# 10258392511/InverseProblemWithDiffusionModel

Hardware: AMD Instinct MI355X
Metric: ALD reconstructions/sec (128x128 complex, R=40, 4-coil) (higher is better)
Workload: dtype f32 (convolutions: operands as two fp16 pieces = 22 significand bits + 2 signs, three fp16 MFMAs per product, fp32 accumulate; every image scaled into fp16's range by an exact power of two from its producer's per-image maxima: any fp32 input, DESIGN.md 4.2); 1 GPU; ACDC-style 128x128 complex SENSE R=40 4-coil ALD reconstruction, NCSNv2Deepest ngf=128 (94.1M params, seeded random init), sigma 348->0.01 x 2311 levels x 3 steps, L2Penalty, denoise; 14 posterior samples = 14 on rank 0 + 13 per further rank (the 105-sample / 8-GPU partition of BASELINE config 3); samples_total=14, samples_this_rank=14, parallelism=sample-sharded x1, hip_graph=True, state_finite=True

## Files before the change

include/ipdm.h:

```cpp
#ifndef IPDM_H
#define IPDM_H

#include <stddef.h>
#include <stdint.h>

#ifdef __cplusplus
extern "C" {
#endif

#define IPDM_OK 0
#define IPDM_EINVAL (-1)
#define IPDM_EUNSUPPORTED (-2)

#define IPDM_ACT_NONE 0
#define IPDM_ACT_ELU 1
#define IPDM_ACT_RELU 2
#define IPDM_ACT_LRELU02 3
#define IPDM_ACT_SWISH 4
#define IPDM_ACT_COPY 5

#define IPDM_AMAX_WAYS 8
#define IPDM_AMAX_SLOT 128

#define IPDM_ABI_VERSION 4
// ... 235 lines not shown
int ipdm_ndft_forward_sets_c64(const float* x, const float* sens, const double* traj, int traj_sets, float* y, float* work,
                               int B, int n_coils, int M, int H, int W, void* stream);
int ipdm_ndft_adjoint_sets_c64(const float* y, const float* sens, const double* traj, int traj_sets, const float* weights,
                               float* x, float* work, int B, int n_coils, int M, int H, int W, void* stream);
int ipdm_toeplitz_psf_sets_f32(const double* traj, int traj_sets, const float* weights, float* psf, float* work, int M, int H,
                               int W, void* stream);
int ipdm_toeplitz_normal_sets_c64(const float* v, const float* sens, const float* psf, int psf_sets, float* out, float* work,
                                  int B, int n_coils, int H, int W, void* stream);
int ipdm_nc_sense_cgprox_sets_f32(const float* z_re, const float* z_im, const float* sens, const float* psf, int psf_sets,
                                  float a, const float* ahy, int max_iter, float tol, float* out_re, float* out_im,
                                  float* work, int32_t* iters_out, int B, int n_coils, int H, int W, void* stream);
int ipdm_ald_nc_sense_cg_step_sets_f32(float* x_re, float* x_im, const float* g_re, const float* g_im,
                                       const float* noise_re, const float* noise_im,
                                       float step, float noise_scale, uint64_t seed, int64_t sample_offset, int64_t step_id,
                                       const ipdm_sched_t* dev_sched, int sched_stride, const float* sens, const float* psf,
                                       int psf_sets, float coef, float* work, const float* ahy, int max_iter, float tol,
                                       int32_t* iters_out, int B, int n_coils, int H, int W, void* stream);

size_t ipdm_nc_coil_gram_workspace_bytes(int B, int n_coils, int M);
int ipdm_nc_coil_gram_c64(const float* y, const float* weights, float* gram, float* work, int B, int n_coils, int M, void* stream);

int ipdm_langevin_step_f32(float* x, const float* g, const float* noise, float step, float noise_scale,
                           uint64_t seed, int64_t sample_offset, int64_t step_id, const ipdm_sched_t* dev_sched,
                           int64_t n_samples, int64_t sample_elems, void* stream);

int ipdm_philox_normal_f32(float* out, uint64_t seed, int64_t sample_offset, int64_t step_id, int plane,
                           int64_t n_samples, int64_t sample_elems, void* stream);

int ipdm_philox_block_host(uint64_t seed, int64_t sample, int64_t step_id, int plane, uint32_t quad, uint32_t* out4);


int ipdm_instnorm_plus_coef_f32(const float* x, const float* alpha, const float* gamma, const float* beta,
                                float* coef, int B, int C, int HW,
                                float* amax_bound ,
                                void* stream);
int ipdm_cond_instnorm_plus_coef_f32(const float* x, const float* embed, const int64_t* labels, int num_classes, int bias,
                                     float* coef, int B, int C, int HW, float* amax_bound, void* stream);
int ipdm_affine_act_f32(const float* x, const float* coef, float* y, int B, int C, int HW, int act, void* stream);
int ipdm_act_f32(const float* x, float* y, int64_t n, int act, void* stream);
int ipdm_scale_shift_f32(const float* x, float* y, int64_t n, float a, float b, void* stream);
int ipdm_add_f32(const float* x, const float* y, float* out, int64_t n, void* stream);
int ipdm_div_sigma_f32(const float* x, const float* sigmas, const int64_t* labels, float* out,
                       int B, int64_t sample_elems, void* stream);
int ipdm_conv3x3_thin_supported(int Cin, int Cout, int H, int W);
int ipdm_conv3x3_thin_f32(const float* x, const float* w, const float* bias,
                          const float* coef ,
                          float* out, int B, int Cin, int Cout, int H, int W, void* stream);
int ipdm_conv3x3_thin_stats_partials(int Cin, int Cout, int H, int W);
int ipdm_conv3x3_thin_stats_f32(const float* x, const float* w, const float* bias, const float* coef, float* out, float* part,
                                int B, int Cin, int Cout, int H, int W, void* stream);
int ipdm_conv3x3_fewout_fin_supported(int Cin, int Cout, int H, int W);
int ipdm_conv3x3_fewout_fin_f32(const float* x, const float* w, const float* bias, const float* coef, int act, float* out,
                                int B, int Cin, int Cout, int H, int W, void* stream);
int ipdm_maxpool5_f32(const float* x, float* y, int planes, int H, int W, void* stream);
int ipdm_affine_avgpool5_f32(const float* x, const float* coef, float* y, int planes, int H, int W, void* stream);
int ipdm_meanpool2_f32(const float* x, float* y, int planes, int H, int W, void* stream);
int ipdm_bilinear_f32(const float* x, float* out, int planes, int in_h, int in_w, int out_h, int out_w,
                      int accumulate, int act ,
                      int planes_per_image, float* amax_out ,
                      void* stream);
int ipdm_trilinear_f32(const float* x, float* out, int planes, int in_d, int in_h, int in_w, int out_d, int out_h,
                       int out_w, int accumulate, int act, int planes_per_image, float* amax_out, void* stream);

int ipdm_groupnorm_coef_f32(const float* x, const float* weight, const float* bias, float* coef,
                            int B, int C, int HW, int G, float eps,
                            float* plane_amax ,
                            void* stream);
int ipdm_groupnorm_coef_partials_f32(const float* part1, int C1, const float* part2, int C2, int P, const float* weight,
                                     const float* bias, float* coef , int B, int G, float eps, void* stream);
int ipdm_groupnorm_coef_cat_f32(const float* x1, int C1, const float* x2, int C2, const float* weight, const float* bias,
                                float* coef, int B, int HW, int G, float eps, float* plane_amax ,
                                void* stream);
int ipdm_affine_act_cat_f32(const float* x1, int C1, const float* x2, int C2, const float* coef, float* y, int B, int HW,
                            int act, void* stream);
int ipdm_linear_f32(const float* x, const float* W, const float* bias, float* y, int B, int In, int Out,
                    int act, void* stream);
int ipdm_attention_f32(const float* q, const float* k, const float* v, float* out, int B, int C, int N,
                       float scale, void* stream);
int ipdm_axpby_f32(const float* x, const float* y, float* out, int64_t n, float a, float b, void* stream);
int ipdm_sample_axpy2_f32(const float* x, const float* y, const float* z, const float* a, const float* c,
                          float* out, int n_samples, int64_t sample_elems, void* stream);
int ipdm_sample_norm_f32(const float* x, float* norms, int n_samples, int64_t sample_elems, void* stream);

int ipdm_conv_pack_weight_f32(const float* w , float* wt, int Cout, int Cin, int k, void* stream);
int ipdm_conv2d_f32(const float* x, const float* wt, const float* bias, const float* coef, int act,
                    const float* residual, float* out, float* out_act, int act_out,
                    int B, int Cin, int Cout, int H, int W, int k, int dilation, int pool2, void* stream);

int ipdm_conv_wino_weight_f32(const float* w , float* U, int Cout, int Cin, void* stream);
int ipdm_conv2d_wino_supported(int Cin, int Cout, int H, int W, int dilation);
int ipdm_conv2d_wino_f32(const float* x, const float* U, const float* bias, const float* residual, float* out,
                         float* out_act, int act_out, int B, int Cin, int Cout, int H, int W, int dilation,
                         void* stream);

int ipdm_debug_set_stamp_buffer(void* buf);
int64_t ipdm_debug_lds_optin_count(void);

int ipdm_conv3d_f32(const float* x, const float* wt, const float* bias, const float* coef, int act,
                    const float* residual, float* out, float* out_act, int act_out,
                    int B, int Cin, int Cout, int D, int H, int W, int k, int dilation, void* stream);

int ipdm_maxpool3d5_f32(const float* x, float* y, int planes, int D, int H, int W, void* stream);
int ipdm_temporal_taps_f32(const float* x, float* out, int planes, int S, int T_in, int T_out, int mode, void* stream);

typedef struct {
  const float* in_amax;
// ... 135 lines not shown
```

inverseproblemwithdiffusionmodel_amd/_lib.py:

```python
import ctypes
import os

import torch
from ctypes import c_char_p, c_double, c_float, c_int, c_int64, c_uint64, c_void_p


class ConvExt(ctypes.Structure):
    _fields_ = [("in_amax", c_void_p), ("bias_bstride", c_int), ("out_scale", c_float), ("res_second", c_int),
                ("out_amax", c_void_p), ("act_amax", c_void_p)]


_HERE = os.path.dirname(os.path.abspath(__file__))
LIB_PATH = os.environ.get("IPDM_LIB") or os.path.join(_HERE, "libipdm.so")

P = c_void_p

SIGNATURES = {
    "ipdm_abi_version": [],
    "ipdm_build_arch": [],
    "ipdm_upfirdn2d_f32": [P, P, P] + [c_int] * 14 + [P],
    "ipdm_fused_bias_act_f32": [P, P, P, P, c_int64, c_int, c_int, c_int, c_int, c_float, c_float, P],
    "ipdm_upfirdn2d_f16": [P, P, P] + [c_int] * 14 + [P],
    "ipdm_upfirdn2d_f64": [P, P, P] + [c_int] * 14 + [P],
    "ipdm_fused_bias_act_f16": [P, P, P, P, c_int64, c_int, c_int, c_int, c_int, c_float, c_float, P],
# ... 59 lines not shown
    "ipdm_ald_singlecoil_step_f32": [P, P, P, P, P, P, c_float, c_float, c_uint64, c_int64, c_int64, P,
                                     P, P, c_int, c_float, c_int, P, c_int, c_int, c_int, P],
    "ipdm_pc_langevin_coef_workspace_bytes": [c_int],
    "ipdm_pc_langevin_coef_f32": [P, P, P, P, c_double, c_double, c_uint64, c_int64, c_int64, P, c_float, c_float, P, P,
                                  c_int, c_int64, P],
    "ipdm_pc_sense_step_f32": [P, P, P, P, P, P, c_float, c_float, c_uint64, c_int64, c_int64, P, c_int,
                               P, P, c_int, c_int, P, c_int, c_float, P, c_int, c_int, c_int, c_int, P],
    "ipdm_pc_sense_cg_step_f32": [P, P, P, P, P, P, c_float, c_float, c_uint64, c_int64, c_int64, P, c_int,
                                  P, P, c_int, c_int, P, c_int, c_float, P, P, c_int, c_float, P,
                                  c_int, c_int, c_int, c_int, P],
    "ipdm_pc_singlecoil_step_f32": [P, P, P, P, P, P, c_float, c_float, c_uint64, c_int64, c_int64, P, c_int,
                                    P, P, c_int, c_float, c_int, P, c_int, c_int, c_int, P],
    "ipdm_nc_supported": [c_int, c_int],
    "ipdm_ndft_workspace_bytes": [c_int, c_int, c_int],
    "ipdm_ndft_forward_c64": [P, P, P, P, P, c_int, c_int, c_int, c_int, c_int, P],
    "ipdm_ndft_adjoint_c64": [P, P, P, P, P, P, c_int, c_int, c_int, c_int, c_int, P],
    "ipdm_toeplitz_psf_workspace_bytes": [c_int, c_int, c_int],
    "ipdm_toeplitz_psf_f32": [P, P, P, P, c_int, c_int, c_int, P],
    "ipdm_toeplitz_workspace_bytes": [c_int, c_int, c_int, c_int],
    "ipdm_toeplitz_normal_c64": [P, P, P, P, P, c_int, c_int, c_int, c_int, P],
    "ipdm_nc_sense_cg_workspace_bytes": [c_int, c_int, c_int, c_int],
    "ipdm_nc_sense_cgprox_f32": [P, P, P, P, c_float, P, c_int, c_float, P, P, P, P, c_int, c_int, c_int, c_int, P],
    "ipdm_ald_nc_sense_cg_step_f32": [P, P, P, P, P, P, c_float, c_float, c_uint64, c_int64, c_int64, P, c_int,
                                      P, P, c_float, P, P, c_int, c_float, P, c_int, c_int, c_int, c_int, P],
    "ipdm_ndft_forward_sets_c64": [P, P, P, c_int, P, P, c_int, c_int, c_int, c_int, c_int, P],
    "ipdm_ndft_adjoint_sets_c64": [P, P, P, c_int, P, P, P, c_int, c_int, c_int, c_int, c_int, P],
    "ipdm_toeplitz_psf_sets_f32": [P, c_int, P, P, P, c_int, c_int, c_int, P],
    "ipdm_toeplitz_normal_sets_c64": [P, P, P, c_int, P, P, c_int, c_int, c_int, c_int, P],
    "ipdm_nc_sense_cgprox_sets_f32": [P, P, P, P, c_int, c_float, P, c_int, c_float, P, P, P, P, c_int, c_int, c_int, c_int, P],
    "ipdm_ald_nc_sense_cg_step_sets_f32": [P, P, P, P, P, P, c_float, c_float, c_uint64, c_int64, c_int64, P, c_int,
                                           P, P, c_int, c_float, P, P, c_int, c_float, P, c_int, c_int, c_int, c_int, P],
    "ipdm_nc_coil_gram_workspace_bytes": [c_int, c_int, c_int],
    "ipdm_nc_coil_gram_c64": [P, P, P, P, c_int, c_int, c_int, P],
    "ipdm_langevin_step_f32": [P, P, P, c_float, c_float, c_uint64, c_int64, c_int64, P, c_int64, c_int64, P],
    "ipdm_philox_normal_f32": [P, c_uint64, c_int64, c_int64, c_int, c_int64, c_int64, P],
    "ipdm_philox_block_host": [c_uint64, c_int64, c_int64, c_int, ctypes.c_uint32, P],
    "ipdm_instnorm_plus_coef_f32": [P, P, P, P, P, c_int, c_int, c_int, P, P],
    "ipdm_cond_instnorm_plus_coef_f32": [P, P, P, c_int, c_int, P, c_int, c_int, c_int, P, P],
    "ipdm_affine_act_f32": [P, P, P, c_int, c_int, c_int, c_int, P],
    "ipdm_act_f32": [P, P, c_int64, c_int, P],
    "ipdm_scale_shift_f32": [P, P, c_int64, c_float, c_float, P],
    "ipdm_add_f32": [P, P, P, c_int64, P],
    "ipdm_div_sigma_f32": [P, P, P, P, c_int, c_int64, P],
    "ipdm_maxpool5_f32": [P, P, c_int, c_int, c_int, P],
    "ipdm_affine_avgpool5_f32": [P, P, P, c_int, c_int, c_int, P],
    "ipdm_meanpool2_f32": [P, P, c_int, c_int, c_int, P],
    "ipdm_bilinear_f32": [P, P, c_int, c_int, c_int, c_int, c_int, c_int, c_int, c_int, P, P],
    "ipdm_conv3x3_thin_supported": [c_int, c_int, c_int, c_int],
    "ipdm_conv3x3_thin_f32": [P, P, P, P, P, c_int, c_int, c_int, c_int, c_int, P],
    "ipdm_conv3x3_thin_stats_partials": [c_int, c_int, c_int, c_int],
    "ipdm_conv3x3_thin_stats_f32": [P, P, P, P, P, P, c_int, c_int, c_int, c_int, c_int, P],
    "ipdm_conv3x3_fewout_fin_supported": [c_int, c_int, c_int, c_int],
    "ipdm_conv3x3_fewout_fin_f32": [P, P, P, P, c_int, P, c_int, c_int, c_int, c_int, c_int, P],
    "ipdm_trilinear_f32": [P, P, c_int, c_int, c_int, c_int, c_int, c_int, c_int, c_int, c_int, c_int, P, P],
    "ipdm_groupnorm_coef_f32": [P, P, P, P, c_int, c_int, c_int, c_int, c_float, P, P],
    "ipdm_groupnorm_coef_partials_f32": [P, c_int, P, c_int, c_int, P, P, P, c_int, c_int, c_float, P],
    "ipdm_groupnorm_coef_cat_f32": [P, c_int, P, c_int, P, P, P, c_int, c_int, c_int, c_float, P, P],
    "ipdm_affine_act_cat_f32": [P, c_int, P, c_int, P, P, c_int, c_int, c_int, P],
    "ipdm_linear_f32": [P, P, P, P, c_int, c_int, c_int, c_int, P],
    "ipdm_attention_f32": [P, P, P, P, c_int, c_int, c_int, c_float, P],
    "ipdm_axpby_f32": [P, P, P, c_int64, c_float, c_float, P],
    "ipdm_sample_axpy2_f32": [P, P, P, P, P, P, c_int, c_int64, P],
    "ipdm_sample_norm_f32": [P, P, c_int, c_int64, P],
    "ipdm_conv_pack_weight_f32": [P, P, c_int, c_int, c_int, P],
    "ipdm_conv2d_f32": [P, P, P, P, c_int, P, P, P, c_int] + [c_int] * 8 + [P],
    "ipdm_conv_wino_weight_f32": [P, P, c_int, c_int, P],
    "ipdm_conv2d_wino_supported": [c_int, c_int, c_int, c_int, c_int],
    "ipdm_conv2d_wino_f32": [P, P, P, P, P, P, c_int, c_int, c_int, c_int, c_int, c_int, c_int, P],
    "ipdm_debug_set_stamp_buffer": [P],
    "ipdm_debug_lds_optin_count": [],
    "ipdm_conv3d_f32": [P, P, P, P, c_int, P, P, P, c_int] + [c_int] * 8 + [P],
    "ipdm_maxpool3d5_f32": [P, P, c_int, c_int, c_int, c_int, P],
    "ipdm_temporal_taps_f32": [P, P, c_int, c_int, c_int, c_int, c_int, P],
    "ipdm_conv_bx3_weight_bytes": [c_int, c_int, c_int],
    "ipdm_conv_bx3_pack_weight": [P, P, c_int, c_int, c_int, P],
    "ipdm_conv2d_bx3_f32": [P, P, P, P, c_int, P, P, P, c_int] + [c_int] * 7 + [P, P],
    "ipdm_conv3d_bx3_f32": [P, P, P, P, c_int, P, P, P, c_int] + [c_int] * 8 + [P, P],
    "ipdm_conv_bx3_splitk": [c_int] * 8,
    "ipdm_conv_bx3_splitk_f32": [P, P, P, P, c_int, P, P, P, c_int] + [c_int] * 10 + [P, P, P],
    "ipdm_adam_ascent_f32": [P, P, P, P, c_int64, c_float, c_float, c_float, c_float, c_int, P],
    "ipdm_conv_wino_bx3_weight_bytes": [c_int, c_int],
    "ipdm_conv_wino_bx3_pack_weight": [P, P, c_int, c_int, P],
    "ipdm_conv2d_wino_bx3_supported": [c_int, c_int, c_int, c_int, c_int],
    "ipdm_conv2d_wino_bx3_f32": [P, P, P, P, P, P, c_int, c_int, c_int, c_int, c_int, c_int, c_int, c_int, P, P],
    "ipdm_conv2d_wino_bx3_stats_partials": [c_int, c_int, c_int, c_int, c_int, c_int],
    "ipdm_conv2d_wino_bx3_splitk": [c_int, c_int, c_int, c_int, c_int],
    "ipdm_conv2d_wino_bx3_splitk_f32": [P, P, P, P, P, P, c_int, c_int, c_int, c_int, c_int, c_int, c_int, c_int, P, P, P],
    "ipdm_conv2d_wino_bx3_stats_f32": [P, P, P, P, P, P, c_int, c_int, c_int, c_int, c_int, c_int, c_int, c_int, P, P, P],
    "ipdm_conv_hx2_weight_bytes": [c_int, c_int, c_int],
    "ipdm_conv_hx2_pack_weight": [P, P, c_int, c_int, c_int, P],
    "ipdm_absmax_f32": [P, P, c_int, c_int64, P],
    "ipdm_conv2d_hx2_f32": [P, P, P, P, c_int, P, P, P, c_int] + [c_int] * 7 + [P, P],
    "ipdm_conv3d_hx2_f32": [P, P, P, P, c_int, P, P, P, c_int] + [c_int] * 8 + [P, P],
    "ipdm_conv_hx2_splitk_f32": [P, P, P, P, c_int, P, P, P, c_int] + [c_int] * 10 + [P, P, P],
    "ipdm_conv_wino_hx2_weight_bytes": [c_int, c_int],
    "ipdm_conv_wino1d_weight_bytes": [c_int, c_int],
    "ipdm_conv_wino1d_pack_weight": [P, P, c_int, c_int, P],
    "ipdm_conv2d_wino1d_supported": [c_int, c_int, c_int, c_int],
    "ipdm_conv_wino1d_weight_bytes3d": [c_int, c_int],
    "ipdm_conv_wino1d_pack_weight3d": [P, P, c_int, c_int, P],
    "ipdm_conv3d_wino1d_supported": [c_int, c_int, c_int, c_int, c_int],
    "ipdm_conv3d_wino1d_f32": [P, P, P, P, P, P, c_int, c_int, c_int, c_int, c_int, c_int, c_int, P, P],
    "ipdm_conv2d_wino1d_f32": [P, P, P, P, c_int, P, P, P, c_int, c_int, c_int, c_int, c_int, c_int, c_int, P, P],
    "ipdm_conv2d_wino1d_stats_partials": [c_int, c_int, c_int, c_int],
    "ipdm_conv2d_wino1d_stats_f32": [P, P, P, P, c_int, P, P, P, c_int, c_int, c_int, c_int, c_int, c_int, c_int, P, P, P],
    "ipdm_conv_wino_hx2_pack_weight": [P, P, c_int, c_int, P],
    "ipdm_conv2d_wino_hx2_f32": [P, P, P, P, P, P, c_int, c_int, c_int, c_int, c_int, c_int, c_int, c_int, P, P],
    "ipdm_conv2d_wino_hx2_form": [c_int] * 5,
    "ipdm_conv2d_wino_hx2_splitk_f32": [P, P, P, P, P, P, c_int, c_int, c_int, c_int, c_int, c_int, c_int, c_int, P, P, P],
    "ipdm_conv2d_wino_hx2_stats_f32": [P, P, P, P, P, P, c_int, c_int, c_int, c_int, c_int, c_int, c_int, c_int, P, P, P],
    "ipdm_instnorm_plus_coef_partials_f32": [P, c_int, P, P, P, P, c_int, c_int, c_int, P, P],
    "ipdm_cond_instnorm_plus_coef_partials_f32": [P, c_int, P, P, c_int, c_int, P, c_int, c_int, c_int, P, P],
    "ipdm_conv1d_hx2_supported": [c_int] * 5,
    "ipdm_conv1d_hx2_weight_bytes": [c_int, c_int, c_int],
    "ipdm_conv1d_hx2_pack_weight": [P, P, c_int, c_int, c_int, P],
    "ipdm_conv1d_hx2_f32": [P, P, P, P, P, P, c_int] + [c_int] * 7 + [P, P],
    "ipdm_meanpool1d2_f32": [P, P, c_int, c_int, P],
    "ipdm_scale_shift_amax_f32": [P, P, P, c_int, c_int64, c_float, c_float, P],
    "ipdm_zero_insert2_f32": [P, P, c_int, c_int, c_int, P],
    "ipdm_subsample2_f32": [P, P, c_int, c_int, c_int, c_int, c_int, c_int, c_int, P],
    "ipdm_in_prelu_fwd_f32": [P, P, P, P, P, c_int, c_int, c_float, P],
    "ipdm_in_prelu_bwd_f32": [P, P, P, P, P, c_int, c_int, P],
    "ipdm_in_prelu_bwd_eps_f32": [P, P, P, P, P, c_int, c_int, c_float, P],
    "ipdm_seg_loglh_grad_f32": [P, P, P, c_int, c_int, c_int64, P],
    "ipdm_axpy_sched_f32": [P, P, P, c_int64, P, c_float, c_int64, P],
    "ipdm_magnitude_c64": [P, P, c_int64, P],
    "ipdm_posterior_moments_c64": [P, P, c_int, c_int64, P],
    "ipdm_tv_c64": [P, P, c_int, c_int, c_int, P],
    "ipdm_tv_grad_c64": [P, P, c_int, c_int, c_int, P],
    "ipdm_nrmse_f32": [P, P, P, c_int, c_int64, c_int, P],
    "ipdm_ssim_f32": [P, P, P, c_int, c_int, c_int, c_int, ctypes.c_double, P],
}
_RESTYPES = {"ipdm_build_arch": c_char_p, "ipdm_debug_lds_optin_count": c_int64, "ipdm_fft2c_workspace_bytes": c_int64, "ipdm_sense_workspace_bytes": c_int64, "ipdm_sense_cg_workspace_bytes": c_int64,
             "ipdm_pc_langevin_coef_workspace_bytes": c_int64,
             "ipdm_ndft_workspace_bytes": c_int64, "ipdm_toeplitz_psf_workspace_bytes": c_int64,
             "ipdm_toeplitz_workspace_bytes": c_int64, "ipdm_nc_sense_cg_workspace_bytes": c_int64,
             "ipdm_conv_bx3_weight_bytes": c_int64,
             "ipdm_conv_wino_bx3_weight_bytes": c_int64, "ipdm_conv_hx2_weight_bytes": c_int64,
             "ipdm_conv_wino_hx2_weight_bytes": c_int64, "ipdm_conv_wino1d_weight_bytes": c_int64, "ipdm_conv_wino1d_weight_bytes3d": c_int64,
             "ipdm_conv1d_hx2_weight_bytes": c_int64, "ipdm_csm_workspace_bytes": ctypes.c_size_t,
             "ipdm_coilcomp_workspace_bytes": ctypes.c_size_t, "ipdm_gcc_workspace_bytes": ctypes.c_size_t,
             "ipdm_espirit_workspace_bytes": ctypes.c_size_t, "ipdm_nc_coil_gram_workspace_bytes": ctypes.c_size_t}

IPDM_EINVAL = -1
IPDM_EUNSUPPORTED = -2


class IpdmError(RuntimeError):
    pass


class IpdmUnsupported(IpdmError, NotImplementedError):
    pass


def _load():
    if not os.path.exists(LIB_PATH):
        raise ImportError(
            f"{LIB_PATH} is missing: the HIP kernels are not built. Run `python -c 'import __graft_entry__ as g; "
            "g.build()'` (or inverseproblemwithdiffusionmodel_amd/csrc/build.py). There is no CPU fallback.")
    lib = ctypes.CDLL(LIB_PATH)
    for name, argtypes in SIGNATURES.items():
        fn = getattr(lib, name)
        fn.argtypes = argtypes
        fn.restype = _RESTYPES.get(name, c_int)
    return lib


lib = _load()


def check(rc, what):
    if rc == 0:
        return
    if rc == IPDM_EUNSUPPORTED:
        raise IpdmUnsupported(f"{what}: no gfx950 kernel for this size/combination (IPDM_EUNSUPPORTED)")
    if rc == IPDM_EINVAL:
        raise IpdmError(f"{what}: invalid argument (IPDM_EINVAL)")
    raise IpdmError(f"{what}: HIP error {rc}")


def call(name, *args):
    check(getattr(lib, name)(*args), name)
```

inverseproblemwithdiffusionmodel_amd/ncsn/models/layers.py:

```python
import os
from functools import partial

import torch
import torch.nn as nn

from ... import ops, _lib
from .normalization import InstanceNorm2dPlus, ConditionalInstanceNorm2dPlus, get_normalization


class _Act:

    def __init__(self, name):
        self.name = name
        self.code = ops.ACT_CODES[name]

    def __call__(self, x):
        return ops.act(x, self.code)


USE_WINOGRAD = os.environ.get("IPDM_WINOGRAD", "1") != "0"
FUSE_POOL = os.environ.get("IPDM_FUSE_POOL", "1") != "0"


def get_act(config):
# ... 99 lines not shown
            if thin_stats:
                return ops.conv3x3_thin(x, self.weight.data, bias, coef, want_stats=True)
            return ops.conv3x3_thin(x, self.weight.data, bias, coef)
        if route == ops.ROUTE_WINO_F32:
            return ops.conv2d_wino(x, self.packed_wino(), bias, residual, act_out=act_out, raw=raw,
                                   dilation=self.dilation)
        if route in (ops.ROUTE_WINO1D, ops.ROUTE_WINO_SPLIT):
            return ops.conv2d_wino_bx3(x, self.packed_wino1d() if route == ops.ROUTE_WINO1D else self.packed_wino_bx3(), bias, residual,
                                       act_out=act_out, raw=raw, dilation=self.dilation, want_stats=want_stats, in_amax=in_amax,
                                       want_amax=produce, res_second=res_second)
        if route == ops.ROUTE_WINO1D_VOL:
            return ops.conv3d(x, self._cached("wino1d_vol", ops.conv_wino1d_weight3d), bias, residual=residual, **tail)
        if route == ops.ROUTE_DIRECT3D:
            return ops.conv3d(x, self.packed(), bias, coef, act, residual, self.dilation, **tail)
        return ops.conv2d(x, self.packed(), bias, coef, act, residual, self.dilation, out=out, **tail)


def conv1x1(in_planes, out_planes, stride=1, bias=True, spec_norm=False, ndim=2):
    assert stride == 1 and not spec_norm
    return Conv2d(in_planes, out_planes, 1, bias=bias, ndim=ndim)


def conv3x3(in_planes, out_planes, stride=1, bias=True, spec_norm=False, ndim=2):
    assert stride == 1 and not spec_norm
    return Conv2d(in_planes, out_planes, 3, bias=bias, ndim=ndim)


def dilated_conv3x3(in_planes, out_planes, dilation, bias=True, spec_norm=False, ndim=2):
    assert not spec_norm
    return Conv2d(in_planes, out_planes, 3, dilation=dilation, bias=bias, ndim=ndim)


def _maxpool(x):
    if x.dim() == 3:
        return ops.maxpool1d5(x)
    return ops.maxpool3d5(x) if x.dim() == 5 else ops.maxpool5(x)


class ConvMeanPool(nn.Module):
    def __init__(self, input_dim, output_dim, kernel_size=3, biases=True, adjust_padding=False, spec_norm=False, ndim=2):
        super().__init__()
        if adjust_padding or spec_norm:
            raise NotImplementedError("adjust_padding / spec_norm are unused by every shipped config")
        if ndim == 3:
            raise NotImplementedError("the 8-way 3-D ConvMeanPool is unused by NCSN3DShallow (all its stages are dilated)")
        self.conv = Conv2d(input_dim, output_dim, kernel_size, bias=biases, ndim=ndim)

    def forward(self, inputs, feeds_conv=True):
        if self.conv.ndim == 1:
            if self.conv.kernel_size == 1:
                return self.conv(ops.meanpool1d2(inputs), feeds_conv=feeds_conv)
            return ops.meanpool1d2(self.conv(inputs, feeds_conv=feeds_conv))
        if self.conv.kernel_size == 1:
            return self.conv(ops.meanpool2(inputs), feeds_conv=feeds_conv)
        return ops.meanpool2(self.conv(inputs, feeds_conv=feeds_conv))

    def fused(self, inputs, residual=None, act_out=ops.ACT_NONE, feeds_conv=True, coef=None, act=ops.ACT_NONE):
        c = self.conv
        route = c.route(inputs, site="pool", coef=coef, act=act, act_out=act_out)
        bias, dyn = None if c.bias is None else c.bias.data, ops.dynamic_range()
        if route is None:
            return None
        if route == ops.ROUTE_SEQ:
            return ops.conv1d(inputs, c.packed_conv1d(), bias, residual, c.dilation,
                              act_out=act_out, in_amax=ops.in_amax_for(inputs) if dyn else None, want_amax=dyn and feeds_conv,
                              pool2=True)
        try:
            if coef is not None:
                return ops.conv2d_wino_bx3(inputs, c.packed_wino1d(), bias, residual,
                                           act_out=act_out, pool2=True, want_stats=True,
                                           in_amax=getattr(coef, "_ipdm_amax_bound", None) if dyn else None,
                                           want_amax=dyn and feeds_conv, coef=coef, act=act)
            return ops.conv2d_wino_bx3(inputs, c.packed_wino1d() if route == ops.ROUTE_WINO1D else c.packed_wino_bx3(), bias, residual,
                                       act_out=act_out, pool2=True, want_stats=True,
                                       in_amax=ops.in_amax_for(inputs), want_amax=dyn and feeds_conv)
        except _lib.IpdmUnsupported:
            return None


class CRPBlock(nn.Module):
    def __init__(self, features, n_stages, act=None, maxpool=True, spec_norm=False, ndim=2):
        super().__init__()
        if not maxpool:
            raise NotImplementedError("average-pool CRP is unused by every shipped config")
        self.convs = nn.ModuleList([conv3x3(features, features, bias=False, spec_norm=spec_norm, ndim=ndim)
                                    for _ in range(n_stages)])
        self.n_stages = n_stages
        self.act = act

    def forward(self, x, x_act=None, want_act=False):
        code = _act_code(self.act)
        x = x_act if x_act is not None else ops.act(x, code)
        path, out_act = x, None
        for i in range(self.n_stages):
            pooled = _maxpool(path)
            if i == self.n_stages - 1:
                if want_act:
                    x, out_act = self.convs[i](pooled, residual=x, act_out=code)
                else:
                    x = self.convs[i](pooled, residual=x)
            elif ops.split_impl():
                path, x = self.convs[i](pooled, residual=x, res_second=True, act_out=ops.ACT_COPY)
            else:
                path = self.convs[i](pooled)
                x = ops.add(path, x)
        return x, out_act
# ... 346 lines not shown
```

inverseproblemwithdiffusionmodel_amd/ops.py:

```python
import ctypes
import os

import torch

from . import _lib
from ._lib import call, P

ACT_NONE, ACT_ELU, ACT_RELU, ACT_LRELU02, ACT_SWISH = 0, 1, 2, 3, 4
ACT_COPY = 5
CONV_TRACE = None

ACT_CODES = {"none": ACT_NONE, None: ACT_NONE, "elu": ACT_ELU, "relu": ACT_RELU, "lrelu": ACT_LRELU02,
             "swish": ACT_SWISH}


def _gpu(t, dtype=None, name="tensor"):
    if not isinstance(t, torch.Tensor) or not t.is_cuda:
        raise RuntimeError(f"ipdm: {name} must be a GPU tensor (the HIP path has no CPU fallback); got "
                           f"{getattr(t, 'device', type(t))}")
    if dtype is not None and t.dtype != dtype:
        raise TypeError(f"ipdm: {name} must be {dtype}, got {t.dtype}")
    return t if t.is_contiguous() else t.contiguous()


# ... 1944 lines not shown
    x = _gpu(x, torch.float32, "x")
    B, Cin, H, W = x.shape
    kk, Cin_w, Cout = wt.shape
    if Cin_w != Cin:
        raise ValueError(f"conv2d: weight Cin {Cin_w} != input Cin {Cin}")
    k = {1: 1, 9: 3}[kk]
    oh, ow = (H // 2, W // 2) if pool2 else (H, W)
    out, out_act, _, _ = _conv_outputs(x, (B, Cout, oh, ow), raw, act_out, "conv2d", out)
    e0 = _trace_open()
    call("ipdm_conv2d_f32", _ptr(x), _ptr(wt), _ptr(bias), _ptr(coef), act, _ptr(residual), _ptr(out), _ptr(out_act),
         act_out, B, Cin, Cout, H, W, k, dilation, int(bool(pool2)), _stream())
    _written(out)
    return _conv_done(e0, out, out_act, B=B, Cin=Cin, Cout=Cout, H=H, W=W, k=k, dil=dilation, res=residual is not None)


USE_THIN_CONV = os.environ.get("IPDM_THIN_CONV", "1") != "0"


def conv3x3_thin_ok(Cin, Cout, H, W, x=None):
    if x is not None and x.data_ptr() % 16:
        return False
    return USE_THIN_CONV and bool(_lib.lib.ipdm_conv3x3_thin_supported(int(Cin), int(Cout), int(H), int(W)))


THIN_STATS = os.environ.get("IPDM_THIN_STATS", "1") != "0"
THIN_FIN = os.environ.get("IPDM_THIN_FIN", "1") != "0"
END_STATS = os.environ.get("IPDM_END_STATS", "1") != "0"


def conv3x3_thin_stats_ok(Cin, Cout, H, W, x=None):
    return (THIN_STATS and USE_STATS_EPILOGUE and conv3x3_thin_ok(Cin, Cout, H, W, x)
            and int(_lib.lib.ipdm_conv3x3_thin_stats_partials(int(Cin), int(Cout), int(H), int(W))) > 0)


def conv3x3_fewout_fin_ok(Cin, Cout, H, W, x, act=ACT_ELU):
    return (THIN_FIN and act == ACT_ELU and x.dim() == 4 and Cout <= 3 < Cin and conv3x3_thin_ok(Cin, Cout, H, W, x)
            and bool(_lib.lib.ipdm_conv3x3_fewout_fin_supported(int(Cin), int(Cout), int(H), int(W))))


def conv3x3_fewout_fin(x, weight, bias, coef, act=ACT_ELU):
    x = _gpu(x, torch.float32, "x")
    weight = _gpu(weight, torch.float32, "weight")
    coef = _gpu(coef, torch.float32, "coef")
    B, Cin, H, W = x.shape
    Cout = weight.shape[0]
    if tuple(weight.shape) != (Cout, Cin, 3, 3):
        raise ValueError(f"conv3x3_fewout_fin: weight {tuple(weight.shape)} does not match input channels {Cin}")
    if tuple(coef.shape) != (B, Cin, 3):
        raise ValueError(f"conv3x3_fewout_fin: coef {tuple(coef.shape)} != {(B, Cin, 3)}")
    out = torch.empty((B, Cout, H, W), dtype=torch.float32, device=x.device)
    e0 = _trace_open()
    call("ipdm_conv3x3_fewout_fin_f32", _ptr(x), _ptr(weight), _ptr(bias), _ptr(coef), act, _ptr(out), B, Cin, Cout, H, W, _stream())
    return _conv_done(e0, out, None, B=B, Cin=Cin, Cout=Cout, H=H, W=W, k=3, dil=1, res=False, thin=True, fin=True)


def conv3x3_thin(x, weight, bias=None, coef=None, want_stats=False):
    x = _gpu(x, torch.float32, "x")
    weight = _gpu(weight, torch.float32, "weight")
    B, Cin, H, W = x.shape
    Cout = weight.shape[0]
    if tuple(weight.shape) != (Cout, Cin, 3, 3):
        raise ValueError(f"conv3x3_thin: weight {tuple(weight.shape)} does not match input channels {Cin}")
    out = torch.empty((B, Cout, H, W), dtype=torch.float32, device=x.device)
    e0 = _trace_open()
    if coef is not None:
        coef = _gpu(coef, torch.float32, "coef")
        if tuple(coef.shape) != (B, Cin, 3):
            raise ValueError(f"conv3x3_thin: coef {tuple(coef.shape)} != {(B, Cin, 3)}")
    if want_stats and conv3x3_thin_stats_ok(Cin, Cout, H, W, x):
        P = int(_lib.lib.ipdm_conv3x3_thin_stats_partials(Cin, Cout, H, W))
        part = torch.empty((B, Cout, P, 3), dtype=torch.float32, device=x.device)
        call("ipdm_conv3x3_thin_stats_f32", _ptr(x), _ptr(weight), _ptr(bias), _ptr(coef), _ptr(out), _ptr(part), B, Cin, Cout, H, W,
             _stream())
        out._ipdm_partials = (part, (out._version, out.data_ptr()))
        return _conv_done(e0, out, None, B=B, Cin=Cin, Cout=Cout, H=H, W=W, k=3, dil=1, res=False, thin=True, stats=True)
    call("ipdm_conv3x3_thin_f32", _ptr(x), _ptr(weight), _ptr(bias), _ptr(coef), _ptr(out), B, Cin, Cout, H, W, _stream())
    return _conv_done(e0, out, None, B=B, Cin=Cin, Cout=Cout, H=H, W=W, k=3, dil=1, res=False, thin=True)


CONV_IMPL = os.environ.get("IPDM_CONV_IMPL", "hx2")
SPLIT_IMPLS = ("hx2", "bx3")
if CONV_IMPL not in SPLIT_IMPLS + ("f32",):
    raise ValueError(f"IPDM_CONV_IMPL={CONV_IMPL!r}: expected 'hx2', 'bx3' or 'f32'")


def split_impl():
    return CONV_IMPL in SPLIT_IMPLS


def impl_unbounded():
    env = os.environ.get("IPDM_CONV_IMPL_UNBOUNDED")
    if env:
        if env not in SPLIT_IMPLS + ("f32",):
            raise ValueError(f"IPDM_CONV_IMPL_UNBOUNDED={env!r}")
        return env
    return CONV_IMPL


def unbounded_amax():
    return True if impl_unbounded() == "hx2" else None


class PackedWeightCache:

    def __init__(self):
        self._entries = {}
# ... 475 lines not shown
```

Measured before the change: 0.1221 reconstructions/s.

## Fuse 2x2 mean-pool into a streaming persistent 1x1 conv for downsampling shortcuts

Adds a persistent HIP kernel that reads the full-resolution input, averages 2x2 blocks in registers, splits the result into fp16 hi/lo pieces in LDS, and runs a three-MFMA 1x1 conv with weights staged in LDS. It replaces the separate meanpool2 pass followed by a 1x1 conv in the downsampling shortcut path. The goal is to skip writing and re-reading the pooled intermediate and to save a launch. It brings in a new weight packing format, grouped accumulation to limit fp32 error, and a prefetch pipeline whose efficiency for these small shapes is uncertain.

```diff
diff --git a/include/ipdm.h b/include/ipdm.h
--- a/include/ipdm.h
+++ b/include/ipdm.h
@@ -311,6 +311,11 @@
 int ipdm_conv3x3_fewout_fin_supported(int Cin, int Cout, int H, int W);
 int ipdm_conv3x3_fewout_fin_f32(const float* x, const float* w, const float* bias, const float* coef, int act, float* out,
                                 int B, int Cin, int Cout, int H, int W, void* stream);
+int ipdm_conv1x1_pool2_supported(int Cin, int Cout, int H, int W);
+int64_t ipdm_conv1x1_pool2_weight_bytes(int Cout, int Cin);
+int ipdm_conv1x1_pool2_pack_weight(const float* w, void* packed, int Cout, int Cin, void* stream);
+int ipdm_conv1x1_pool2_f32(const float* x, const void* wq, const float* bias, const float* in_amax, float* out, int B, int Cin,
+                           int Cout, int H, int W, void* stream);
 int ipdm_maxpool5_f32(const float* x, float* y, int planes, int H, int W, void* stream);
 int ipdm_affine_avgpool5_f32(const float* x, const float* coef, float* y, int planes, int H, int W, void* stream);
 int ipdm_meanpool2_f32(const float* x, float* y, int planes, int H, int W, void* stream);
diff --git a/inverseproblemwithdiffusionmodel_amd/_lib.py b/inverseproblemwithdiffusionmodel_amd/_lib.py
--- a/inverseproblemwithdiffusionmodel_amd/_lib.py
+++ b/inverseproblemwithdiffusionmodel_amd/_lib.py
@@ -135,6 +135,10 @@
     "ipdm_conv3x3_thin_stats_f32": [P, P, P, P, P, P, c_int, c_int, c_int, c_int, c_int, P],
     "ipdm_conv3x3_fewout_fin_supported": [c_int, c_int, c_int, c_int],
     "ipdm_conv3x3_fewout_fin_f32": [P, P, P, P, c_int, P, c_int, c_int, c_int, c_int, c_int, P],
+    "ipdm_conv1x1_pool2_supported": [c_int, c_int, c_int, c_int],
+    "ipdm_conv1x1_pool2_weight_bytes": [c_int, c_int],
+    "ipdm_conv1x1_pool2_pack_weight": [P, P, c_int, c_int, P],
+    "ipdm_conv1x1_pool2_f32": [P, P, P, P, P, c_int, c_int, c_int, c_int, c_int, P],
     "ipdm_trilinear_f32": [P, P, c_int, c_int, c_int, c_int, c_int, c_int, c_int, c_int, c_int, c_int, P, P],
     "ipdm_groupnorm_coef_f32": [P, P, P, P, c_int, c_int, c_int, c_int, c_float, P, P],
     "ipdm_groupnorm_coef_partials_f32": [P, c_int, P, c_int, c_int, P, P, P, c_int, c_int, c_float, P],
@@ -221,7 +225,7 @@
              "ipdm_conv_bx3_weight_bytes": c_int64,
              "ipdm_conv_wino_bx3_weight_bytes": c_int64, "ipdm_conv_hx2_weight_bytes": c_int64,
              "ipdm_conv_wino_hx2_weight_bytes": c_int64, "ipdm_conv_wino1d_weight_bytes": c_int64, "ipdm_conv_wino1d_weight_bytes3d": c_int64,
-             "ipdm_conv1d_hx2_weight_bytes": c_int64, "ipdm_csm_workspace_bytes": ctypes.c_size_t,
+             "ipdm_conv1d_hx2_weight_bytes": c_int64, "ipdm_conv1x1_pool2_weight_bytes": c_int64, "ipdm_csm_workspace_bytes": ctypes.c_size_t,
              "ipdm_coilcomp_workspace_bytes": ctypes.c_size_t, "ipdm_gcc_workspace_bytes": ctypes.c_size_t,
              "ipdm_espirit_workspace_bytes": ctypes.c_size_t, "ipdm_nc_coil_gram_workspace_bytes": ctypes.c_size_t}
 
diff --git a/inverseproblemwithdiffusionmodel_amd/csrc/conv1x1_stream.hip b/inverseproblemwithdiffusionmodel_amd/csrc/conv1x1_stream.hip
--- /dev/null
+++ b/inverseproblemwithdiffusionmodel_amd/csrc/conv1x1_stream.hip
@@ -0,0 +1,296 @@
+#include "conv_kernel.h"
+
+namespace {
+
+using namespace ipdm_conv;
+
+constexpr int S1_PX = 64;
+constexpr int S1_KG = 8;
+constexpr int S1_STAGE = 512;
+constexpr int S1_SC = 2 * S1_STAGE;
+constexpr int S1_W = S1_SC + 256;
+constexpr size_t S1_LDS_BASE = (size_t)S1_W * 16;
+constexpr size_t S1_LDS_MAX = 160 * 1024;
+
+struct S1Args {
+  const float* x;
+  const uint4* wq;
+  const float* bias;
+  const float* in_amax;
+  float* out;
+  int Cin, Cout, H, W;
+  int tpi, ntiles;
+};
+
+template <int NCTW, int D, bool WLDS, bool GROUPED>
+__global__ __launch_bounds__(512, 1) void conv1x1_pool2_kernel(S1Args a) {
+  extern __shared__ __align__(16) uint4 s1_lds[];
+  const int tid = threadIdx.x, lane = tid & 63, wave = tid >> 6;
+  const int h = lane >> 5, j = lane & 31;
+  const int OW = a.W >> 1, OHW = (a.H >> 1) * OW;
+  const size_t HW = (size_t)a.H * a.W;
+  const int n_cc = a.Cin >> 4, n_ct = a.Cout >> 5, nks = (n_cc + 1) >> 1;
+  const int G = (int)gridDim.x;
+  const int my_tiles = (int)blockIdx.x < a.ntiles ? (a.ntiles - 1 - (int)blockIdx.x) / G + 1 : 0;
+
+  float* const sc_lds = reinterpret_cast<float*>(s1_lds + S1_SC);
+  {
+    const float* winv = reinterpret_cast<const float*>(a.wq + (size_t)n_cc * n_ct * 128);
+    if (tid < a.Cout) {
+      sc_lds[tid] = winv[tid];
+      sc_lds[512 + tid] = a.bias ? a.bias[tid] : 0.f;
+    }
+    if constexpr (WLDS) {
+      const int nfr = n_cc * n_ct * 128;
+      for (int i = tid; i < nfr; i += 512) s1_lds[S1_W + i] = a.wq[i];
+    }
+  }
+  __syncthreads();
+
+  const int sub = tid >> 8, cp = (tid >> 5) & 7, pp = tid & 31;
+  auto tile_ptr = [&](int tile) __attribute__((always_inline)) {
+    const int b = tile / a.tpi, tp = tile - b * a.tpi;
+    int op = tp * S1_PX + 2 * pp;
+    op = op < OHW ? op : OHW - 2;
+    const int oy = op / OW, ox = op - oy * OW;
+    return a.x + ((size_t)b * a.Cin + sub * 16 + 2 * cp) * HW + (size_t)(2 * oy) * a.W + 2 * ox;
+  };
+  int ld_tile = (int)blockIdx.x, ld_ks = 0;
+  long long ld_rem = (long long)my_tiles * nks;
+  const float* ld_ptr = my_tiles ? tile_ptr(ld_tile) : a.x;
+  auto issue = [&](float4 (&r)[4]) __attribute__((always_inline)) {
+    if (ld_rem <= 0) return;
+    if (ld_ks * 32 + sub * 16 < a.Cin) {
+      const float* p = ld_ptr + (size_t)ld_ks * 32 * HW;
+      r[0] = *reinterpret_cast<const float4*>(p);
+      r[1] = *reinterpret_cast<const float4*>(p + a.W);
+      r[2] = *reinterpret_cast<const float4*>(p + HW);
+      r[3] = *reinterpret_cast<const float4*>(p + HW + a.W);
+    }
+    --ld_rem;
+    if (++ld_ks == nks) {
+      ld_ks = 0;
+      ld_tile += G;
+      if (ld_rem > 0) ld_ptr = tile_ptr(ld_tile);
+    }
+  };
+
+  const int pt = wave & 1, ctb = wave >> 1;
+  f32x16 acc[NCTW];
+  [[maybe_unused]] f32x16 tot[GROUPED ? NCTW : 1];
+#pragma unroll
+  for (int i = 0; i < NCTW; ++i)
+#pragma unroll
+    for (int r = 0; r < 16; ++r) {
+      acc[i][r] = 0.f;
+      if constexpr (GROUPED) tot[i][r] = 0.f;
+    }
+
+  int c_tile = (int)blockIdx.x, c_ks = 0, cb = 0, ctp = 0;
+  float hx_in = 1.f, hx_out = 1.f;
+  unsigned* const lds32 = reinterpret_cast<unsigned*>(s1_lds);
+
+  auto step = [&](float4 (&r)[4], int par) __attribute__((always_inline)) {
+    if (c_ks == 0) {
+      cb = __builtin_amdgcn_readfirstlane(c_tile / a.tpi);
+      ctp = c_tile - cb * a.tpi;
+      hx_in = hx_out = 1.f;
+      if (a.in_amax) hx_dynamic_scale(ipdm_amax_read(a.in_amax + (size_t)cb * IPDM_AMAX_SLOT), hx_in, hx_out);
+    }
+    const int cc0 = c_ks * 2;
+    const bool two = cc0 + 1 < n_cc;
+    constexpr int ASETS = NCTW < 4 ? 2 : 1;
+    [[maybe_unused]] uint4 afr[ASETS][NCTW][2];
+    [[maybe_unused]] auto load_A = [&](uint4 (&fr)[NCTW][2], int cc) __attribute__((always_inline)) {
+#pragma unroll
+      for (int i = 0; i < NCTW; ++i) {
+        const int ct = ctb + 4 * i < n_ct ? ctb + 4 * i : n_ct - 1;
+        const uint4* p = a.wq + ((size_t)cc * n_ct + ct) * 128 + lane;
+        fr[i][0] = p[0];
+        fr[i][1] = p[64];
+      }
+    };
+    if constexpr (!WLDS) {
+      load_A(afr[0], cc0);
+      if constexpr (ASETS == 2) load_A(afr[1], two ? cc0 + 1 : cc0);
+    }
+    if (sub == 0 || two) {
+      const float m00 = (((r[0].x + r[1].x) + r[0].y) + r[1].y) * 0.25f, m01 = (((r[0].z + r[1].z) + r[0].w) + r[1].w) * 0.25f;
+      const float m10 = (((r[2].x + r[3].x) + r[2].y) + r[3].y) * 0.25f, m11 = (((r[2].z + r[3].z) + r[2].w) + r[3].w) * 0.25f;
+      unsigned* st = lds32 + par * (S1_STAGE * 4) + sub * 1024 + ((cp >> 2) * 64 + 2 * pp) * 4 + (cp & 3);
+      unsigned hp, lp;
+      split2_pk_scaled(m00, m10, hx_in, hp, lp);
+      st[0] = hp;
+      st[512] = lp;
+      split2_pk_scaled(m01, m11, hx_in, hp, lp);
+      st[4] = hp;
+      st[516] = lp;
+    }
+    issue(r);
+    __syncthreads();
+    const uint4* cur = s1_lds + par * S1_STAGE + h * 64 + pt * 32 + j;
+#pragma unroll
+    for (int sb = 0; sb < 2; ++sb) {
+      if (sb == 0 || two) {
+        const f16x8 bh = __builtin_bit_cast(f16x8, cur[sb * 256]), bl = __builtin_bit_cast(f16x8, cur[sb * 256 + 128]);
+        if constexpr (!WLDS && ASETS == 1) {
+          if (sb == 1) load_A(afr[0], cc0 + 1);
+        }
+#pragma unroll
+        for (int i = 0; i < NCTW; ++i) {
+          if (ctb + 4 * i < n_ct) {
+            uint4 fh, fl;
+            if constexpr (WLDS) {
+              const uint4* p = s1_lds + S1_W + ((cc0 + sb) * n_ct + ctb + 4 * i) * 128 + lane;
+              fh = p[0];
+              fl = p[64];
+            } else {
+              fh = afr[sb % ASETS][i][0];
+              fl = afr[sb % ASETS][i][1];
+            }
+            const f16x8 ah = __builtin_bit_cast(f16x8, fh), al = __builtin_bit_cast(f16x8, fl);
+            f32x16 c = acc[i];
+            c = __builtin_amdgcn_mfma_f32_32x32x16_f16(al, bh, c, 0, 0, 0);
+            c = __builtin_amdgcn_mfma_f32_32x32x16_f16(ah, bl, c, 0, 0, 0);
+            c = __builtin_amdgcn_mfma_f32_32x32x16_f16(ah, bh, c, 0, 0, 0);
+            acc[i] = c;
+          }
+        }
+      }
+    }
+    if constexpr (GROUPED) {
+      if (((c_ks + 1) & (S1_KG / 2 - 1)) == 0 || c_ks + 1 == nks) {
+#pragma unroll
+        for (int i = 0; i < NCTW; ++i)
+#pragma unroll
+          for (int rr = 0; rr < 16; ++rr) {
+            tot[i][rr] += acc[i][rr];
+            acc[i][rr] = 0.f;
+          }
+      }
+    }
+    if (++c_ks == nks) {
+      const int px = ctp * S1_PX + pt * 32 + j;
+#pragma unroll
+      for (int i = 0; i < NCTW; ++i) {
+        const int ct = ctb + 4 * i;
+        if (ct < n_ct) {
+          float* op = a.out + ((size_t)cb * a.Cout + ct * 32 + 4 * h) * OHW + px;
+#pragma unroll
+          for (int rr = 0; rr < 16; ++rr) {
+            const int dco = (rr & 3) + 8 * (rr >> 2);
+            const int co = ct * 32 + 4 * h + dco;
+            float sum;
+            if constexpr (GROUPED) {
+              sum = tot[i][rr];
+              tot[i][rr] = 0.f;
+            } else {
+              sum = acc[i][rr];
+              acc[i][rr] = 0.f;
+            }
+            const float v = fmaf(sum, sc_lds[co] * hx_out, sc_lds[512 + co]);
+            if (px < OHW) op[(size_t)dco * OHW] = v;
+          }
+        }
+      }
+      c_ks = 0;
+      c_tile += G;
+    }
+  };
+
+  float4 xr[D][4];
+  static_for<D>([&](auto dc) { issue(xr[decltype(dc)::value]); });
+  const long long total = (long long)my_tiles * nks;
+  for (long long s0 = 0; s0 < total; s0 += D) {
+    static_for<D>([&](auto dc) {
+      constexpr int d = decltype(dc)::value;
+      if (s0 + d < total) step(xr[d], (int)((s0 + d) & 1));
+    });
+  }
+}
+
+__global__ __launch_bounds__(256) void s1_pack_kernel(const float* __restrict__ w, unsigned short* __restrict__ out,
+                                                      float* __restrict__ inv_scale, int Cout, int Cin, int n_ct) {
+  __shared__ float red[256];
+  const int co = blockIdx.x, tid = threadIdx.x;
+  float m = 0.f;
+  for (int i = tid; i < Cin; i += 256) m = fmaxf(m, fabsf(w[(int64_t)co * Cin + i]));
+  red[tid] = m;
+  __syncthreads();
+  for (int st = 128; st > 0; st >>= 1) {
+    if (tid < st) red[tid] = fmaxf(red[tid], red[tid + st]);
+    __syncthreads();
+  }
+  int e = 0;
+  const float mx = red[0];
+  const bool ok = mx > 0.f && mx < INFINITY;
+  if (ok) (void)frexpf(mx, &e);
+  const float inv = ok ? ldexpf(1.f, e - 14) : 1.f;
+  if (tid == 0) inv_scale[co] = inv;
+  const int ct = co >> 5, r = co & 31;
+  for (int ci = tid; ci < Cin; ci += 256) {
+    const float v = w[(int64_t)co * Cin + ci] * (1.f / inv);
+    const _Float16 hi = (_Float16)v;
+    const _Float16 lo = (_Float16)(v - (float)hi);
+    const int64_t base = ((int64_t)(ci >> 4) * n_ct + ct) * 1024 + ((ci >> 3) & 1) * 256 + r * 8 + (ci & 7);
+    out[base] = __builtin_bit_cast(unsigned short, hi);
+    out[base + 512] = __builtin_bit_cast(unsigned short, lo);
+  }
+}
+
+template <int NCTW, int D, bool GROUPED>
+int s1_launch_g(const S1Args& a, bool wlds, unsigned grid, hipStream_t s) {
+  if (wlds)
+    return ipdm_launch_lds(conv1x1_pool2_kernel<NCTW, D, true, GROUPED>, dim3(grid), dim3(512),
+                           S1_LDS_BASE + (size_t)a.Cin * a.Cout * 4, s, a);
+  return ipdm_launch_lds(conv1x1_pool2_kernel<NCTW, D, false, GROUPED>, dim3(grid), dim3(512), S1_LDS_BASE, s, a);
+}
+template <int NCTW, int D>
+int s1_launch(const S1Args& a, bool wlds, unsigned grid, hipStream_t s) {
+  return a.Cin > 16 * S1_KG ? s1_launch_g<NCTW, D, true>(a, wlds, grid, s) : s1_launch_g<NCTW, D, false>(a, wlds, grid, s);
+}
+
+}
+
+extern "C" int ipdm_conv1x1_pool2_supported(int Cin, int Cout, int H, int W) {
+  return (Cin > 0 && Cout > 0 && H > 0 && W > 0 && H % 2 == 0 && W % 8 == 0 && Cin % 16 == 0 && Cout % 32 == 0 && Cin <= 512 &&
+          Cout <= 512)
+             ? 1
+             : 0;
+}
+
+extern "C" int64_t ipdm_conv1x1_pool2_weight_bytes(int Cout, int Cin) {
+  if (Cout <= 0 || Cin <= 0 || Cin % 16 || Cout % 32 || Cin > 512 || Cout > 512) return -1;
+  return (int64_t)(Cin / 16) * (Cout / 32) * 2048 + (int64_t)Cout * 4;
+}
+
+extern "C" int ipdm_conv1x1_pool2_pack_weight(const float* w, void* packed, int Cout, int Cin, void* stream) {
+  IPDM_REQUIRE(w && packed && Cout > 0 && Cin > 0);
+  if (ipdm_conv1x1_pool2_weight_bytes(Cout, Cin) < 0) return IPDM_EUNSUPPORTED;
+  const int n_cc = Cin / 16, n_ct = Cout / 32;
+  float* inv_scale = reinterpret_cast<float*>(static_cast<char*>(packed) + (int64_t)n_cc * n_ct * 2048);
+  hipLaunchKernelGGL(s1_pack_kernel, dim3(Cout), dim3(256), 0, ipdm_stream(stream), w, (unsigned short*)packed, inv_scale, Cout,
+                     Cin, n_ct);
+  return ipdm_launch_status();
+}
+
+extern "C" int ipdm_conv1x1_pool2_f32(const float* x, const void* wq, const float* bias, const float* in_amax, float* out, int B,
+                                      int Cin, int Cout, int H, int W, void* stream) {
+  IPDM_REQUIRE(B >= 0 && Cin > 0 && Cout > 0 && H > 0 && W > 0);
+  if (!ipdm_conv1x1_pool2_supported(Cin, Cout, H, W)) return IPDM_EUNSUPPORTED;
+  if (B == 0) return IPDM_OK;
+  IPDM_REQUIRE(x && wq && out && x != out);
+  if ((reinterpret_cast<uintptr_t>(x) & 15) != 0 || (reinterpret_cast<uintptr_t>(wq) & 15) != 0) return IPDM_EUNSUPPORTED;
+  const int OHW = (H / 2) * (W / 2);
+  const int tpi = (OHW + S1_PX - 1) / S1_PX;
+  const int64_t ntiles = (int64_t)B * tpi;
+  if (ntiles > 0x3fffffff) return IPDM_EUNSUPPORTED;
+  S1Args a{x, static_cast<const uint4*>(wq), bias, in_amax, out, Cin, Cout, H, W, tpi, (int)ntiles};
+  static const int wlds_on = ipdm_env_int("IPDM_S1_WLDS", 1);
+  const bool wlds = wlds_on && S1_LDS_BASE + (size_t)Cin * Cout * 4 <= S1_LDS_MAX;
+  const unsigned grid = ipdm_persistent_grid(ntiles);
+  hipStream_t s = ipdm_stream(stream);
+  if (Cout <= 128) return s1_launch<1, 3>(a, wlds, grid, s);
+  if (Cout <= 256) return s1_launch<2, 3>(a, wlds, grid, s);
+  return s1_launch<4, 2>(a, wlds, grid, s);
+}
diff --git a/inverseproblemwithdiffusionmodel_amd/ncsn/models/layers.py b/inverseproblemwithdiffusionmodel_amd/ncsn/models/layers.py
--- a/inverseproblemwithdiffusionmodel_amd/ncsn/models/layers.py
+++ b/inverseproblemwithdiffusionmodel_amd/ncsn/models/layers.py
@@ -175,6 +175,12 @@
                 return self.conv(ops.meanpool1d2(inputs), feeds_conv=feeds_conv)
             return ops.meanpool1d2(self.conv(inputs, feeds_conv=feeds_conv))
         if self.conv.kernel_size == 1:
+            c = self.conv
+            bias = None if c.bias is None else c.bias.data
+            if (c.ndim == 2 and not feeds_conv and inputs.dim() == 4
+                    and ops.conv1x1_pool2_ok(c.in_planes, c.out_planes, inputs.shape[2], inputs.shape[3], inputs, bias)):
+                return ops.conv1x1_pool2(inputs, c._cached("stream1x1", ops.conv1x1_pool2_weight), bias,
+                                         in_amax=ops.in_amax_for(inputs))
             return self.conv(ops.meanpool2(inputs), feeds_conv=feeds_conv)
         return ops.meanpool2(self.conv(inputs, feeds_conv=feeds_conv))
 
diff --git a/inverseproblemwithdiffusionmodel_amd/ops.py b/inverseproblemwithdiffusionmodel_amd/ops.py
--- a/inverseproblemwithdiffusionmodel_amd/ops.py
+++ b/inverseproblemwithdiffusionmodel_amd/ops.py
@@ -2020,6 +2020,53 @@
     e0 = _trace_open()
     call("ipdm_conv3x3_fewout_fin_f32", _ptr(x), _ptr(weight), _ptr(bias), _ptr(coef), act, _ptr(out), B, Cin, Cout, H, W, _stream())
     return _conv_done(e0, out, None, B=B, Cin=Cin, Cout=Cout, H=H, W=W, k=3, dil=1, res=False, thin=True, fin=True)
+
+
+SHORTCUT_STREAM = os.environ.get("IPDM_SHORTCUT_STREAM", "1") != "0"
+
+
+def conv1x1_pool2_ok(Cin, Cout, H, W, x, bias=None, impl=None):
+    return (SHORTCUT_STREAM and USE_THIN_CONV and (CONV_IMPL if impl is None else impl) == "hx2" and x.dim() == 4
+            and x.is_contiguous() and x.data_ptr() % 16 == 0 and (bias is None or bias.dim() == 1)
+            and bool(_lib.lib.ipdm_conv1x1_pool2_supported(int(Cin), int(Cout), int(H), int(W))))
+
+
+def conv1x1_pool2_weight(w):
+    w = _gpu(w, torch.float32, "weight")
+    Cout, Cin = int(w.shape[0]), int(w.shape[1])
+    if w.numel() != Cout * Cin:
+        raise ValueError(f"conv1x1_pool2_weight: {tuple(w.shape)} is not a 1x1 kernel")
+    nbytes = _lib.lib.ipdm_conv1x1_pool2_weight_bytes(Cout, Cin)
+    if nbytes < 0:
+        raise _lib.IpdmUnsupported(f"conv1x1_pool2_weight: Cin {Cin} / Cout {Cout} outside the streaming kernel's set")
+    blob = torch.empty(nbytes, dtype=torch.uint8, device=w.device)
+    call("ipdm_conv1x1_pool2_pack_weight", _ptr(w), _ptr(blob), Cout, Cin, _stream())
+    return PackedBx3(blob, Cout, Cin, 1, "stream1x1")
+
+
+def conv1x1_pool2(x, packed, bias=None, in_amax=None):
+    x = _gpu(x, torch.float32, "x")
+    if not isinstance(packed, PackedBx3) or packed.fmt != "stream1x1":
+        raise TypeError("conv1x1_pool2: weights must come from conv1x1_pool2_weight")
+    B, Cin, H, W = x.shape
+    if packed.Cin != Cin:
+        raise ValueError(f"conv1x1_pool2: weight Cin {packed.Cin} != input Cin {Cin}")
+    Cout = packed.Cout
+    if bias is not None:
+        bias = _gpu(bias, torch.float32, "bias")
+        if tuple(bias.shape) != (Cout,):
+            raise _lib.IpdmUnsupported(f"conv1x1_pool2: bias {tuple(bias.shape)}: per-channel [{Cout}] or none")
+    if not _lib.lib.ipdm_conv1x1_pool2_supported(Cin, Cout, H, W) or x.data_ptr() % 16:
+        raise _lib.IpdmUnsupported(f"conv1x1_pool2: {Cin} -> {Cout} on {H} x {W} (or an x off a 16-byte boundary) is not served")
+    if in_amax is not None:
+        if (tuple(in_amax.shape) != (B, AMAX_SLOT) or in_amax.dtype != torch.float32 or not in_amax.is_cuda
+                or not in_amax.is_contiguous()):
+            raise ValueError(f"in_amax: expected a maxima vector -- contiguous float32 GPU tensor [{B}, {AMAX_SLOT}]")
+    out = torch.empty((B, Cout, H // 2, W // 2), dtype=torch.float32, device=x.device)
+    e0 = _trace_open()
+    call("ipdm_conv1x1_pool2_f32", _ptr(x), _ptr(packed.blob), _ptr(bias), _ptr(in_amax), _ptr(out), B, Cin, Cout, H, W, _stream())
+    return _conv_done(e0, out, None, B=B, Cin=Cin, Cout=Cout, H=H // 2, W=W // 2, k=1, dil=1, bx3=True, fmt="hx2", res=False,
+                      taps3d=None)
 
 
 def conv3x3_thin(x, weight, bias=None, coef=None, want_stats=False):
```

New measurement: 0.1232 reconstructions/s, median of 6. No clear change (+0.8%).
